# rayanirban/DiffSplitting

Measured on AMD Instinct MI355X. Metric: sampled images/sec (2000-step 128x128 SR3), higher is better.
Workload: dtype bf16; 1 GPU; sr_sr3_16_128: GaussianDiffusion.p_sample_loop, 16->128 SR3 UNet (97.8M params), T=2000 linear schedule; one step = UNet forward + posterior update of the batch; batch_per_gpu=16, global_batch=16, image=128x128x3, sample_steps=2000, parallelism=1 independent replicas, final RCCL all-gather, hipgraph=True, streams=1, noise=device Philox4x32-10, weights=random-init, seed 0

## Files before the change

diffsplitting_amd/csrc/dsx_conv_variants.h:

```cpp
#pragma once
#include "dsx_conv_common.h"

#ifndef DSX_RING_DEPTH
#define DSX_RING_DEPTH 6
#endif
#ifndef DSX_WS_DEPTH_EXPR
#define DSX_WS_DEPTH_EXPR (bm == 64 ? 5 : (bm == 256 ? 2 : (ks == 1 ? 3 : 4)))
#endif
#ifndef DSX_WS_DEPTH_C2_64
#define DSX_WS_DEPTH_C2_64 3
#endif
#ifndef DSX_RING_1X1_NB1
#define DSX_RING_1X1_NB1 16
#endif
#ifndef DSX_RING_1X1_NB2
#define DSX_RING_1X1_NB2 4
#endif

namespace dsx {

template <typename DT, int MB, int WM, int WN, int KS, int S, int CPG, int D, int MAX_IT>
__global__ __launch_bounds__(256, ((KS == 3 && CPG == 2) ? 2
                                  : (MB == 1 ? (S == 2 ? 3 : 4) : (MB == 2 ? 3 : (MB == 4 ? 2 : 1))))) void k_conv_mfma(const ConvArgs a);
template <typename DT, int MB, int WM, int WN, int NB, int KS, int CPG, int D, int NIT, int P, int LW>
__global__ __launch_bounds__(256 + 64 * LW, 1) void k_conv_ws(const ConvArgs a);
template <typename DT, int KS, int NPH> __global__ __launch_bounds__(512, 1) void k_conv_img(const ConvArgs a);

enum ConvFamily { FAM_MFMA, FAM_WS, FAM_IMG };
struct ConvVariant {
  int family, dtype, tile, ks, stride, cpg;
  void (*kern)(const ConvArgs);
  int block, lds_cap;
  int MB, WM, WN, NB;
  int max_px;
  int nit;
  int depth, nbuf;
  bool fuses_stats;
};
static constexpr int kLdsDefault = 64 * 1024, kLdsMax = 160 * 1024;
static constexpr int conv_cpg(int ks) { return ks == 1 ? 2 : 1; }

static constexpr int mfma_max_px(int bm, int ks, int stride, int cpg) {
  if (ks == 1) return bm;
  if (stride == 2) return 400;
  if (cpg == 2) return bm == 256 ? 324 : 220;
  return bm == 256 ? 400 : (bm == 128 ? 220 : 144);
}
template <typename DT, int TILE, int MB, int WM, int WN, int KS, int S = 1, int CPG = conv_cpg(KS)>
constexpr ConvVariant mfma_row() {
  constexpr bool G2 = KS == 3 && CPG == 2;
  constexpr int D = KS == 1 ? 4 : (G2 ? 6 : DSX_RING_DEPTH);
  constexpr int PX = mfma_max_px(32 * MB * WM, KS, S, CPG);
  constexpr int MI = (PX * 4 * CPG + 255) / 256;
  return {FAM_MFMA, Kind<DT>::value, TILE, KS, S, CPG, k_conv_mfma<DT, MB, WM, WN, KS, S, CPG, D, MI>, 256,
          G2 ? kLdsMax : kLdsDefault, MB, WM, WN, 1, PX, MI, 0, 2, MB <= 2};
}

static constexpr int kWsLoaderWaves = 4;
static constexpr int ws_max_px(int bm, int ks) { return ks == 1 ? bm : (bm == 256 ? 324 : (bm == 128 ? 180 : 108)); }
static constexpr int ws_depth(int bm, int ks, int cpg) {
  if (ks == 3 && cpg == 2) return bm == 64 ? DSX_WS_DEPTH_C2_64 : 2;
  if (ks == 3 && cpg == 4) return 1;
  if (ks == 1 && cpg == 4) return bm == 64 ? 2 : 1;
  return DSX_WS_DEPTH_EXPR;
}

#ifndef DSX_WS_NBUF_EXPR
#define DSX_WS_NBUF_EXPR(bm, ks, nb, cpg) ((bm) == 256 && (ks) == 3 ? 3 : 2)
#endif
static constexpr int ws_nbuf(int bm, int ks, int nb, int cpg) { return DSX_WS_NBUF_EXPR(bm, ks, nb, cpg); }

template <typename DT, int TILE, int MB, int WM, int WN, int NB, int KS, int CPG = conv_cpg(KS)>
constexpr ConvVariant ws_row() {
  constexpr int BM = 32 * MB * WM;
  constexpr int D = KS == 1 ? ((NB == 2 || MB == 4) ? DSX_RING_1X1_NB2 : DSX_RING_1X1_NB1) : ((NB == 2 || MB == 4) ? 6 : 18);
  constexpr int PX = ws_max_px(BM, KS);
  constexpr int NIT = (PX * 4 * CPG + kWsLoaderWaves * 64 - 1) / (kWsLoaderWaves * 64);
  constexpr int P = ws_depth(BM, KS, CPG);
  return {FAM_WS, Kind<DT>::value, TILE, KS, 1, CPG, k_conv_ws<DT, MB, WM, WN, NB, KS, CPG, D, NIT, P, kWsLoaderWaves>,
          256 + 64 * kWsLoaderWaves, kLdsMax, MB, WM, WN, NB, PX, NIT, P, ws_nbuf(BM, KS, NB, CPG), true};
}

template <typename DT, int KS, int NPH> constexpr ConvVariant img_row() {
  return {FAM_IMG, Kind<DT>::value, -1, KS, 1, NPH, k_conv_img<DT, KS, NPH>, 512, kLdsMax, 0, 0, 0, 0, 0, 0, 0, 0, true};
}

template <int N> struct ConvVariants {
  ConvVariant row[N];
  constexpr const ConvVariant* begin() const { return row; }
  constexpr const ConvVariant* end() const { return row + N; }
};
template <int... N> constexpr ConvVariants<(N + ...)> concat(const ConvVariants<N>&... parts) {
  ConvVariants<(N + ...)> out{};
  int n = 0;
  auto append = [&](const auto& p) { for (const ConvVariant& v : p) out.row[n++] = v; };
  (append(parts), ...);
  return out;
}

template <typename DT> constexpr ConvVariants<34> variants_of() {
  return {{
      mfma_row<DT, TILE_256x128, 8, 1, 4, 1>(), mfma_row<DT, TILE_256x128, 8, 1, 4, 3>(),
      mfma_row<DT, TILE_128x128, 4, 1, 4, 1>(), mfma_row<DT, TILE_128x128, 4, 1, 4, 3>(),
      mfma_row<DT, TILE_64x128, 2, 1, 4, 1>(), mfma_row<DT, TILE_64x128, 2, 1, 4, 3>(),
      mfma_row<DT, TILE_256x64, 4, 2, 2, 1>(), mfma_row<DT, TILE_256x64, 4, 2, 2, 3>(),
      mfma_row<DT, TILE_128x64, 2, 2, 2, 1>(), mfma_row<DT, TILE_128x64, 2, 2, 2, 3>(),
      mfma_row<DT, TILE_128x64, 2, 2, 2, 3, 1, 2>(),
      mfma_row<DT, TILE_64x64, 1, 2, 2, 1>(), mfma_row<DT, TILE_64x64, 1, 2, 2, 3>(),
      mfma_row<DT, TILE_64x64, 1, 2, 2, 3, 2>(),
      mfma_row<DT, TILE_128x32, 1, 4, 1, 1>(), mfma_row<DT, TILE_128x32, 1, 4, 1, 3>(),
      mfma_row<DT, TILE_128x32, 1, 4, 1, 3, 1, 2>(), mfma_row<DT, TILE_256x32, 2, 4, 1, 3, 1, 2>(),
      ws_row<DT, TILE_64x128, 2, 1, 4, 1, 1>(), ws_row<DT, TILE_64x128, 2, 1, 4, 1, 3>(),
      ws_row<DT, TILE_64x128, 2, 1, 4, 1, 1, 4>(),
      ws_row<DT, TILE_64x128, 2, 1, 4, 1, 3, 2>(),
      ws_row<DT, TILE_64x128, 2, 1, 4, 1, 3, 4>(),
      ws_row<DT, TILE_128x64, 2, 2, 2, 1, 1>(), ws_row<DT, TILE_128x64, 2, 2, 2, 1, 3>(),
      ws_row<DT, TILE_256x64, 4, 2, 2, 1, 3>(),
      ws_row<DT, TILE_64x64, 1, 2, 2, 1, 1>(), ws_row<DT, TILE_64x64, 1, 2, 2, 1, 3>(),
      img_row<DT, 1, 2>(), img_row<DT, 1, 4>(), img_row<DT, 1, 8>(),
      img_row<DT, 3, 2>(), img_row<DT, 3, 4>(), img_row<DT, 3, 8>(),
  }};
}
template <typename DT> constexpr ConvVariants<4> ws_nb2_variants() {
  return {{ws_row<DT, TILE_128x128, 2, 2, 2, 2, 1>(), ws_row<DT, TILE_128x128, 2, 2, 2, 2, 3>(),
           ws_row<DT, TILE_128x128, 2, 2, 2, 2, 1, 4>(), ws_row<DT, TILE_128x128, 2, 2, 2, 2, 3, 2>()}};
}
static constexpr auto kVariants = concat(variants_of<float>(), variants_of<__bf16>(), variants_of<_Float16>(),
                                         ws_nb2_variants<__bf16>(), ws_nb2_variants<_Float16>());

static constexpr int kKeySlots = 3 * 3 * (TILE_COUNT + 1) * 2 * 2 * 4;
static constexpr int key_slot(int family, int dtype, int tile, int ks, int stride, int cpg) {
  const int c = cpg == 1 ? 0 : (cpg == 2 ? 1 : (cpg == 4 ? 2 : (cpg == 8 ? 3 : -1)));
  if (family < 0 || family > FAM_IMG || dtype < 0 || dtype > 2 || tile < -1 || tile >= TILE_COUNT || (ks != 1 && ks != 3) ||
      (stride != 1 && stride != 2) || c < 0)
    return -1;
  return ((((family * 3 + dtype) * (TILE_COUNT + 1) + tile + 1) * 2 + ks / 2) * 2 + stride - 1) * 4 + c;
}
struct VariantIndex { short row[kKeySlots]; bool unique; };
static constexpr VariantIndex index_variants() {
  VariantIndex ix{};
  for (short& r : ix.row) r = -1;
  ix.unique = true;
  short n = 0;
  for (const ConvVariant& v : kVariants) {
    const int s = key_slot(v.family, v.dtype, v.tile, v.ks, v.stride, v.cpg);
    if (s < 0 || ix.row[s] >= 0) ix.unique = false;
    else ix.row[s] = n;
    ++n;
  }
  return ix;
}
static constexpr VariantIndex kIndex = index_variants();
static const ConvVariant* find_variant(int family, int dtype, int tile, int ks, int stride, int cpg) {
  const int s = key_slot(family, dtype, tile, ks, stride, cpg);
  return s >= 0 && kIndex.row[s] >= 0 ? &kVariants.row[kIndex.row[s]] : nullptr;
}

static int patch_pixels(int ks, int stride, const ConvArgs& a) {
  const int TW = 1 << a.tw_log2, TH = 1 << a.th_log2;
  return (((TH - 1) * stride + ks) * ((TW - 1) * stride + ks)) << a.tb_log2;
}
static hipError_t launch_variant(const ConvVariant& v, unsigned grid, size_t lds, const ConvArgs& a, hipStream_t st) {
  void* args[] = {(void*)&a};
  (void)hipLaunchKernel((const void*)v.kern, dim3(grid), dim3((unsigned)v.block), args, lds, st);
  return hipGetLastError();
}

}
```

diffsplitting_amd/csrc/dsx_conv_ws.hip:

```cpp
#include "dsx_conv_variants.h"
#include <algorithm>

#ifndef DSX_PRE_RESID_EXPR
#define DSX_PRE_RESID_EXPR (NB == 1 && MB <= 2)
#endif
#ifndef DSX_PFF_EXPR
#define DSX_PFF_EXPR (NB == 2 ? 3 : 6)
#endif
#ifndef DSX_WS_K0_EXPR
#define DSX_WS_K0_EXPR 64
#endif
#ifndef DSX_EPI_PRIO_COND
#define DSX_EPI_PRIO_COND false
#endif
#ifndef DSX_STAMP_CVT_COND
#define DSX_STAMP_CVT_COND (tiC == 2 && gC == 0)
#endif
#ifndef DSX_LOADER_PRIO
#define DSX_LOADER_PRIO 3
#endif
#ifndef DSX_LOADER_PRIO_EXPR
#define DSX_LOADER_PRIO_EXPR DSX_LOADER_PRIO
#endif

// ... 3 lines not shown
  for (int spin = 0; spin < (1 << 18); ++spin) {
    f32x4_t v;
    asm volatile("ds_read_b128 %0, %1\n\ts_waitcnt lgkmcnt(0)" : "=v"(v) : "v"(addr) : "memory");
    const int4 c = __builtin_bit_cast(int4, v);
    const int m = min(min(c.x, c.y), min(c.z, c.w));
    if (__builtin_amdgcn_readfirstlane(m) >= target) return;
    __builtin_amdgcn_s_sleep(1);
  }
  if (timeouts != nullptr && (threadIdx.x & 63) == 0) atomicAdd(timeouts, 1u);
}
static __device__ __forceinline__ void lds_signal(unsigned addr, int wave, int count) {
  asm volatile("s_waitcnt lgkmcnt(0)" ::: "memory");
  if ((threadIdx.x & 63) == 0) asm volatile("ds_write_b32 %0, %1" ::"v"(addr + 4u * (unsigned)wave), "v"(count) : "memory");
}

template <typename DT, int MB, int WM, int WN, int NB, int KS, int CPG, int D, int NIT, int P, int LW>
__global__ void k_conv_ws(const ConvArgs a) {
  constexpr int LT = 64 * LW;
  constexpr int S = 1;
  constexpr int KC = Chunk<DT>::KC;
  constexpr int CPU = Unit<DT>::N;
  constexpr int ES = (int)sizeof(DT);
  constexpr int UPP = KC / CPU;
  constexpr int UPG = UPP * CPG;
  constexpr int UPG_LOG2 = UPG == 16 ? 4 : (UPG == 8 ? 3 : 2);
  constexpr int UB = 16;
  constexpr int PIXB = 64 * CPG + 16;
  constexpr int TAPS = KS * KS;
  constexpr int PAD = KS / 2;
  constexpr int NSTEP = CPG * TAPS * 2;
  [[maybe_unused]] constexpr bool IS_BF16 = sizeof(DT) == 2;
  constexpr int RAWB = NIT * LT * 16;
  constexpr int NSLOT = P + 1;
  static_assert(D <= NSTEP ? NSTEP % D == 0 : (D % NSTEP == 0 && D / NSTEP <= 8), "ring depth divides the steps per group, or is a multiple of them");
  static_assert(WM * WN == 4 && P * NIT < 64, "4 compute waves; vmcnt is 6 bits");

  extern __shared__ __attribute__((aligned(16))) unsigned char lds[];

  const int tid = threadIdx.x;
  DSX_STAMP_T(63, tid == 0);
  const int lane = tid & 63;
  const int wave8 = __builtin_amdgcn_readfirstlane(tid >> 6);
  const bool loader = wave8 >= 4;
  const int wave = loader ? wave8 - 4 : wave8;
  const int ltid = loader ? tid - 256 : tid;
  const int c16 = lane & 15, kq = lane >> 4;

  const int TW = 1 << a.tw_log2, TH = 1 << a.th_log2;
  const int PW = (TW - 1) * S + KS;
  const int PH = (TH - 1) * S + KS;
  const int PPI = PH * PW;
  const int PP = PPI << a.tb_log2;
  const int RB = a.lds_row;
  const int BUFB = (PH << a.tb_log2) * RB;
  constexpr int NBUF = ws_nbuf(32 * MB * WM, KS, NB, CPG);
  static_assert(NBUF >= 2 && NBUF <= 4, "two images and a barrier, or three / four and counters");
  const int C = a.C0 + a.C1;
  const int AFFB = a.has_gn ? ((2 * C * 4 + 15) & ~15) : 0;
  float* const aff_base = (float*)(lds + NBUF * BUFB);
  unsigned char* const raw_base = lds + NBUF * BUFB + 3 * AFFB;
  const unsigned lds0 = (unsigned)(uintptr_t)(__attribute__((address_space(3))) unsigned char*)lds;
  const unsigned full_addr = lds0 + NBUF * BUFB + 3 * AFFB + NSLOT * RAWB;
  const int G = a.kchunks / CPG;

  const int wpn = a.ws_wg_per_n;
  int nt, p0;
  {
    const int bid = blockIdx.x, xcd = bid & 7, k = bid >> 3;
    if (a.ws_map == 0) {
      const int lg = a.ws_nt_log2, band = xcd >> lg;
      nt = xcd & ((1 << lg) - 1);
// ... 7 lines not shown
      const int j = (int)fastdiv((unsigned)k, a.mg_per);
      nt = k - j * a.ws_per;
      p0 = (j << 3) + xcd;
    } else {
      nt = (int)fastdiv((unsigned)bid, a.mg_wpn);
      p0 = bid - nt * wpn;
    }
  }
  const int ntile = wpn >= a.m_tiles ? (p0 < a.m_tiles ? 1 : 0)
                                     : (a.ws_bigdiv ? (a.m_tiles - p0 + wpn - 1) / wpn
                                                                : (int)fastdiv((unsigned)(a.m_tiles - p0 + wpn - 1), a.mg_wpn));
  const int total = ntile * G;

  if (loader) {
    __builtin_amdgcn_s_setprio(DSX_LOADER_PRIO_EXPR);
    struct TilePos { int tx, ty, b; };
    const int adv_x = a.ws_adv_x, adv_y = a.ws_adv_y, adv_b = a.ws_adv_b;
    auto tile_advance = [&](TilePos& t) __attribute__((always_inline)) {
      t.tx += adv_x;
      if (t.tx >= a.tiles_x) { t.tx -= a.tiles_x; t.ty += 1; }
      t.ty += adv_y;
      if (t.ty >= a.tiles_y) { t.ty -= a.tiles_y; t.b += 1; }
      t.b += adv_b;
    };
    auto tile_flags = [&](const TilePos& t) __attribute__((always_inline)) -> int {
      return (PAD == 0) ? 0
                        : ((t.ty == 0 ? 1 : 0) | (t.ty == a.tiles_y - 1 ? 2 : 0) | (t.tx == 0 ? 4 : 0) |
                           (t.tx == a.tiles_x - 1 ? 8 : 0));
    };
    auto tile_base = [&](const TilePos& t) __attribute__((always_inline)) -> int {
// ... 196 lines not shown
      if (++bufL == NBUF) bufL = 0;
      DSX_STAMP_T(66 + 4 * v, tid == 256 && v < 9);
      if (v + 2 < total) {
        wait_young(issued - (v + 3));
        fetch_next();
      }
      DSX_STAMP_T(67 + 4 * v, tid == 256 && v < 9);
      if constexpr (NBUF == 2) ws_barrier();
      DSX_STAMP_T(68 + 4 * v, tid == 256 && v < 9);
    }
    return;
  }

  const int wm = wave / WN, wn = wave % WN;
  const int pq = ws16_pixel(c16);
  int abase[MB][KS];
#pragma unroll
  for (int mb = 0; mb < MB; ++mb) {
    const int m = (wm * MB + mb) * 32 + pq;
    const int tx = m & (TW - 1);
    const int ty = (m >> a.tw_log2) & (TH - 1);
    const int tb = m >> (a.tw_log2 + a.th_log2);
#pragma unroll
    for (int dy = 0; dy < KS; ++dy)
      abase[mb][dy] = (tb * PH + ty * S + dy) * RB + tx * S * PIXB + ws16_slice(kq) * 16;
  }
  const int a16 = TW >= 32 ? 16 * S * PIXB : (16 >> a.tw_log2) * S * RB;
  const int blk0 = (nt * WN + wn) * NB;
  const int wblock = G * (NSTEP * 1024);
  const __amdgpu_buffer_rsrc_t rsw = __builtin_amdgcn_make_buffer_rsrc(
      (void*)((const unsigned char*)a.wpack + (size_t)blk0 * wblock), 0, NB * wblock, 0x00020000);
  const int wlane[2] = {ws16_woff(lane, 0), ws16_woff(lane, 1)};
  static_assert(D % 2 == 0 && NSTEP % 2 == 0, "ring slots alternate between the two fragments of a pair");
  const int qtot = G * NSTEP;
  int qn = 0;
  struct WFrag { uint4 v[NB]; };
  auto load_b = [&](auto chc) __attribute__((always_inline)) -> WFrag {
    constexpr int ch = decltype(chc)::value;
    WFrag f;
#pragma unroll
    for (int nb = 0; nb < NB; ++nb)
      f.v[nb] = __builtin_bit_cast(uint4, __builtin_amdgcn_raw_buffer_load_b128(rsw, wlane[ch], nb * wblock + (qn >> 1) * 2048, 0));
// ... 40 lines not shown
    return (t.b * a.Ho + (t.ty << a.th_log2)) * a.Wo + (t.tx << a.tw_log2);
  };
  TilePos cur;
  {
    const int q1 = (int)fastdiv((unsigned)p0, a.mg_tiles_x);
    cur.b = (int)fastdiv((unsigned)p0, a.mg_per_img);
    cur.tx = p0 - q1 * a.tiles_x;
    cur.ty = q1 - cur.b * a.tiles_y;
  }
  TilePos nxt = cur;
  tile_advance(nxt);
  TilePos nn = nxt;
  tile_advance(nn);

  auto load_aff = [&](int b, int slot) __attribute__((always_inline)) {
    if (a.gn_scale == nullptr || tid * 4 >= C) return;
    float* dst = aff_base + (size_t)slot * (AFFB / 4);
    *(float4*)(dst + tid * 4) = *(const float4*)(a.gn_scale + (size_t)b * C + tid * 4);
    *(float4*)(dst + C + tid * 4) = *(const float4*)(a.gn_shift + (size_t)b * C + tid * 4);
  };
  TilePos n3 = nn;
  tile_advance(n3);
  load_aff(cur.b, 0);
  if (ntile > 1) load_aff(nxt.b, 1);
  if (ntile > 2) load_aff(nn.b, 2);

  constexpr int NR = 8 / CPU;
  const float4 zero4 = make_float4(0.f, 0.f, 0.f, 0.f);
  float4 addv[NB][2], affv[2];
  constexpr bool PRE_RESID = DSX_PRE_RESID_EXPR;
  uint4 residv[PRE_RESID ? MB : 1][NB][2][NR];
// ... 25 lines not shown
          addv[nb][j] = *(const float4*)(a.film + (size_t)t.b * a.film_bs + nbase + 32 * nb + 4 * j);
    }
    if (PRE_RESID && a.resid) {
      const int r0 = tile_pixel0(t) * a.resid_ld;
#pragma unroll
      for (int mb = 0; mb < (PRE_RESID ? MB : 1); ++mb)
#pragma unroll
        for (int ph = 0; ph < 2; ++ph) {
          const DT* rp = (const DT*)a.resid + (r0 + rrow[mb] + ph * r16);
#pragma unroll
          for (int nb = 0; nb < NB; ++nb)
#pragma unroll
            for (int q = 0; q < NR; ++q) residv[mb][nb][ph][q] = *(const uint4*)(rp + 32 * nb + CPU * q);
        }
    }
    if (want_aff && a.gn_scale != nullptr && tid * 4 < C) {
      affv[0] = *(const float4*)(a.gn_scale + (size_t)b_aff * C + tid * 4);
      affv[1] = *(const float4*)(a.gn_shift + (size_t)b_aff * C + tid * 4);
    }
  };
  prefetch_epilogue(cur, ntile > 3, n3.b);

  constexpr bool PF_OK = !(NB == 2 && KS == 3);
  unsigned fin_pf_acc = 0u;
  if constexpr (PF_OK) fin_pf_acc = l2_prefetch_fold(l2_prefetch(a.pf, blockIdx.x, gridDim.x, tid, 256));
  if constexpr (KS == 1) {
    if (a.fin_on) {
      fin_pf_acc |= l2_prefetch_fold(l2_prefetch(a.fin.pf, blockIdx.x, gridDim.x, tid, 256));
      const int nitems = a.fin.B * a.fin.groups;
      for (int item = (int)blockIdx.x * 4 + wave; item < nitems; item += (int)gridDim.x * 4)
        gn_finalize_item<1>(a.fin, item % a.fin.B, item / a.fin.B, lane, nullptr);
// ... 25 lines not shown
    for (int v0 = 0; v0 < total; v0 += RP)
      static_for<RP>([&](auto rc_) __attribute__((always_inline)) {
        constexpr int R0 = decltype(rc_)::value * NSTEP;
        const int v = v0 + decltype(rc_)::value;
        if (v >= total) return;
#define DSX_WS_ITEM_NEXT return
#include "dsx_conv_ws_item.inc"
#undef DSX_WS_ITEM_NEXT
      });
  }
  if constexpr (PF_OK) l2_prefetch_retire(a.pf, fin_pf_acc);
}

static const ConvVariant* ws_variant(int dtype, int tile, int ks, const ConvArgs& a) {
  const int cpg = (ks == 3 && (a.ws_cpg == 2 || a.ws_cpg == 4)) ? a.ws_cpg : ((ks == 1 && a.ws_cpg == 4) ? 4 : conv_cpg(ks));
  return find_variant(FAM_WS, dtype, tile, ks, 1, cpg);
}
size_t conv_ws_lds_bytes(int dtype, int tile, int ks, const ConvArgs& a) {
  const ConvVariant* v = ws_variant(dtype, tile, ks, a);
  if (!v) return 0;
  const int cpg = v->cpg;
  if (cpg != conv_cpg(ks)) {
    const int gw = cpg * (dtype != 0 ? 32 : 16);
    if ((ks == 3 && a.cpg == 2) || a.kchunks % cpg || a.C0 % gw || a.C1 % gw) return 0;
    if ((1 << (a.tw_log2 + a.th_log2 + a.tb_log2)) != 32 * v->MB * v->WM) return 0;
    if (a.lds_row != conv_lds_row(ks, 1, a.tw_log2, cpg)) return 0;
  } else if (conv_lds_bytes(dtype, tile, ks, 1, a) == 0) return 0;
  if (patch_pixels(ks, 1, a) > v->max_px) return 0;
  if (a.up && (a.tw_log2 == 0 || a.th_log2 == 0)) return 0;
  const int ph = ((1 << a.th_log2) - 1) + ks;
  const size_t bufb = (size_t)(ph << a.tb_log2) * a.lds_row;
  const size_t rawb = (size_t)v->nit * (kWsLoaderWaves * 64 * 16);
  const size_t affb = a.has_gn ? (((size_t)2 * (a.C0 + a.C1) * 4 + 15) & ~(size_t)15) : 0;
  const size_t total = v->nbuf * bufb + 3 * affb + (size_t)(v->depth + 1) * rawb + (v->nbuf >= 3 ? 32 : 0);
  if (a.tb_log2 != 0 || a.kchunks / cpg < 2) return 0;
  if ((long long)a.B * a.Ho * a.Wo * std::max(a.out_ld, a.resid_ld) >= (1LL << 31)) return 0;
  const int al = dtype != 0 ? 7 : 3;
  if (a.Cout % (32 * v->WN * v->NB) != 0 || (a.out_ld & al) != 0 || (a.resid_ld & al) != 0 || a.C0 + a.C1 > 1024)
    return 0;
  if (dtype != 0 && !(a.act_bf16 && a.out_bf16)) return 0;
  return total <= (size_t)v->lds_cap ? total : 0;
}
hipError_t launch_conv_ws(int dtype, int tile, int ks, const ConvArgs& a, hipStream_t st) {
  const size_t lds = conv_ws_lds_bytes(dtype, tile, ks, a);
  if (lds == 0 || a.ksplit != 1 || a.ws_wg_per_n < 1 || a.stage_mode != 0) return hipErrorInvalidValue;
  if (a.bias && a.film) return hipErrorInvalidValue;
  return launch_variant(*ws_variant(dtype, tile, ks, a), (unsigned)(a.n_tiles * a.ws_wg_per_n), lds, a, st);
}

// ... 2 lines not shown
```

diffsplitting_amd/csrc/dsx_conv_ws_item.inc:

```
    unsigned aaddr[MB][KS];
#pragma unroll
    for (int mb = 0; mb < MB; ++mb)
#pragma unroll
      for (int dy = 0; dy < KS; ++dy) aaddr[mb][dy] = lds0 + ibuf * BUFB + abase[mb][dy];
    if constexpr (NBUF >= 3) lds_wait_all_ge(full_addr, v + 1, a.handoff_timeouts);
    f32x4_t fb[PFF + 1];
    auto read_frag = [&](auto kc_) __attribute__((always_inline)) {
      constexpr int k = decltype(kc_)::value;
      constexpr int t = k / NF, mb = (k % NF) >> 1, ph = k & 1;
      constexpr int cg = t / TAPS, tap = t % TAPS, dy = tap / KS, dx = tap % KS;
      constexpr int imm = dx * PIXB + cg * 64;
      static_assert(imm < 65536, "ds offset field");
#ifndef DSX_ABL_L
      lds_read_frag<imm>(fb[k % (PFF + 1)], ph ? aaddr[mb][dy] + (unsigned)a16 : aaddr[mb][dy]);
#else
      touch_frag(fb[k % (PFF + 1)], aaddr[mb][dy]);
#endif
    };
    static_for<PFF>(read_frag);
    static_for<NPAIR>([&](auto tc_) {
      constexpr int t = decltype(tc_)::value;
      constexpr int s0 = (R0 + 2 * t) % D, s1 = (R0 + 2 * t + 1) % D;
      const WFrag w0 = bq[s0], w1 = bq[s1];
#ifndef DSX_ABL_W
      bq[s0] = load_b(std::integral_constant<int, 0>{});
      bq[s1] = load_b(std::integral_constant<int, 1>{});
#endif
      static_for<NF>([&](auto fc_) __attribute__((always_inline)) {
        constexpr int f = decltype(fc_)::value, k = t * NF + f;
        constexpr int mb = f >> 1, ph = f & 1;
        if constexpr (k + PFF < FT) read_frag(std::integral_constant<int, k + PFF>{});
// ... 2 lines not shown
        const f32x4_t px = fb[k % (PFF + 1)];
#pragma unroll
        for (int nb = 0; nb < NB; ++nb) {
          f32x4_t q0 = {acc[mb][nb][8 * ph], acc[mb][nb][8 * ph + 1], acc[mb][nb][8 * ph + 2], acc[mb][nb][8 * ph + 3]};
          f32x4_t q1 = {acc[mb][nb][8 * ph + 4], acc[mb][nb][8 * ph + 5], acc[mb][nb][8 * ph + 6], acc[mb][nb][8 * ph + 7]};
          q0 = mfma16_step<DT>(w0.v[nb], px, q0);
          q1 = mfma16_step<DT>(w1.v[nb], px, q1);
#pragma unroll
          for (int j = 0; j < 4; ++j) { acc[mb][nb][8 * ph + j] = q0[j]; acc[mb][nb][8 * ph + 4 + j] = q1[j]; }
        }
      });
    });
    DSX_STAMP_T(1 + 3 * v, tid == 0 && v < 20);
    if constexpr (NBUF == 2) ws_barrier();
    else lds_signal(full_addr + 16, wave, v + 1);
    if (++ibuf == NBUF) ibuf = 0;
    DSX_STAMP_T(2 + 3 * v, tid == 0 && v < 20);
    if (++g < G) DSX_WS_ITEM_NEXT;
    g = 0;

    if (DSX_EPI_PRIO_COND) __builtin_amdgcn_s_setprio(2);
    if (a.gn_scale != nullptr && ti + 3 < ntile && tid * 4 < C) {
      float* dst = aff_base + (size_t)aslot * (AFFB / 4);
      *(float4*)(dst + tid * 4) = affv[0];
      *(float4*)(dst + C + tid * 4) = affv[1];
    }
    const int rcur = PRE_RESID ? 0 : tile_pixel0(cur) * a.resid_ld;
#pragma unroll
    for (int mb = 0; mb < MB; ++mb)
#pragma unroll
      for (int nb = 0; nb < NB; ++nb)
#pragma unroll
        for (int ph = 0; ph < 2; ++ph) {
          float rs[8];
#pragma unroll
          for (int q = 0; q < NR; ++q) {
            float t[CPU];
// ... 73 lines not shown
```

diffsplitting_amd/csrc/dsx_kernels.h:

```cpp
#pragma once
#include <hip/hip_runtime.h>
#include <stdint.h>

namespace dsx {

struct PrefetchArgs {
  const void* base;
  unsigned slice_bytes;
  int nslices;
  unsigned* sink;
};
inline unsigned fastdiv_magic(unsigned d) { return d <= 1 ? 0u : (unsigned)((1ull << 32) / d) + 1u; }
#if defined(__HIPCC__)
__device__ __forceinline__ unsigned fastdiv(unsigned n, unsigned magic) { return magic ? __umulhi(n, magic) : n; }
struct PfAcc { unsigned v[4]; };
__device__ __forceinline__ PfAcc l2_prefetch(const PrefetchArgs& pf, unsigned lin_block, unsigned nblocks_total, int tid, int nthreads) {
  PfAcc acc = {{0u, 0u, 0u, 0u}};
  if (pf.base == nullptr || pf.nslices <= 0) return acc;
  const unsigned label = lin_block & 7u, j = lin_block >> 3, n8 = (nblocks_total + 7u) >> 3;
  const unsigned lines = pf.slice_bytes >> 7;
  const unsigned per = (lines + n8 - 1u) / n8, l0 = j * per;
  const unsigned l1 = l0 + per < lines ? l0 + per : lines;
  const int s0 = pf.nslices < 8 ? (int)(label % (unsigned)pf.nslices) : (int)label;
  const int sstep = pf.nslices < 8 ? pf.nslices : 8;
// ... 148 lines not shown
  int tiles_x, tiles_y, m_tiles, n_tiles;
  int lds_row;
  int cpg;
  int ws_wg_per_n;
  int ws_cpg;
  int xcd_bands;
  int ws_map;
  int ws_nt_log2;
  int ws_per;
  int ws_adv_x, ws_adv_y, ws_adv_b;
  int ws_dpy, ws_dpx;
  unsigned mg_tiles_x, mg_per_img, mg_pw, mg_wpn, mg_per;
  int ws_bigdiv;
  float* stat_part;
  unsigned* handoff_timeouts;
  unsigned long long* stamp;
  int stamp_block;
  int ablate;
  const void* gn_part0; int gn_nchunk0, gn_pf32_0;
  const void* gn_part1; int gn_nchunk1, gn_pf32_1;
  StatPivot gn_piv0, gn_piv1;
  const float* gn_gamma; const float* gn_beta;
  int gn_groups; float gn_eps;
  PrefetchArgs pf;
  int fin_on;
  GnFinArgs fin;
  int ksplit;
  int groups_per_split;
  long long slab_stride;
};
// ... 395 lines not shown
```

diffsplitting_amd/csrc/dsx_plan.cpp:

```cpp
#include "dsx_rt.h"

static std::vector<int> tile_order(const char* e, const std::vector<int>& dflt) {
  if (!*e) return dflt;
  std::vector<int> v;
  for (const char* p = e; *p;) {
    v.push_back(atoi(p));
    while (*p && *p != ',') ++p;
    if (*p == ',') ++p;
  }
  return v;
}

PlanKnobs dsx::read_plan_knobs() {
  PlanKnobs k;
  static const struct { const char* name; int PlanKnobs::*field; } ints[] = {
      {"DSX_FIRST", &PlanKnobs::first}, {"DSX_IMG", &PlanKnobs::img}, {"DSX_WS", &PlanKnobs::ws},
      {"DSX_WS_1X1", &PlanKnobs::ws_1x1}, {"DSX_WS_MIN_GRID", &PlanKnobs::ws_min_grid}, {"DSX_WS_G2", &PlanKnobs::ws_g2},
      {"DSX_WS_G2_MIN64", &PlanKnobs::ws_g2_min64}, {"DSX_WS_G2_MIN128", &PlanKnobs::ws_g2_min128},
      {"DSX_WS_G4_MIN64", &PlanKnobs::ws_g4_min64}, {"DSX_WS_C4", &PlanKnobs::ws_c4},
      {"DSX_WS_C4_MIN", &PlanKnobs::ws_c4_min}, {"DSX_WS_MAP3", &PlanKnobs::ws_map3},
      {"DSX_XCD_BANDS", &PlanKnobs::xcd_bands}, {"DSX_HOST_FIN", &PlanKnobs::host_fin},
      {"DSX_PREFETCH", &PlanKnobs::prefetch}, {"DSX_PREFETCH_WS", &PlanKnobs::prefetch_ws},
      {"DSX_FUSE_STATS", &PlanKnobs::fuse_stats}, {"DSX_NARROW_G2", &PlanKnobs::narrow_g2},
      {"DSX_MIN_GRID", &PlanKnobs::min_grid}, {"DSX_SPLITK", &PlanKnobs::splitk}, {"DSX_ATTN_CS", &PlanKnobs::attn_cs},
#ifdef DSX_DIAG
      {"DSX_ABLATE", &PlanKnobs::ablate},
#endif
  };
  static const struct { const char* name; std::vector<int> PlanKnobs::*field; } lists[] = {
      {"DSX_TILES_WIDE", &PlanKnobs::tiles_wide}, {"DSX_TILES_NARROW", &PlanKnobs::tiles_narrow},
      {"DSX_TILES_SLIM", &PlanKnobs::tiles_slim}, {"DSX_TILES_WIDE_SPLIT", &PlanKnobs::tiles_wide_split},
      {"DSX_TILES_NARROW_SPLIT", &PlanKnobs::tiles_narrow_split}, {"DSX_TILES_NARROW_G2", &PlanKnobs::tiles_narrow_g2},
      {"DSX_TILES_WS_WIDE", &PlanKnobs::tiles_ws_wide}, {"DSX_TILES_WS_WIDE_1X1", &PlanKnobs::tiles_ws_wide_1x1},
      {"DSX_TILES_WS_WIDE_1X1_RAW", &PlanKnobs::tiles_ws_wide_1x1_raw}, {"DSX_TILES_WS_NARROW", &PlanKnobs::tiles_ws_narrow},
  };
// ... 208 lines not shown
  return wpn;
}

static void decide_ws_chunks(const PlanKnobs& k, int dtype, int ks, int tile, ConvArgs& a) {
  auto take = [&](bool wanted, int cpg) {
    ConvArgs t = a;
    t.ws_cpg = cpg; t.lds_row = conv_lds_row(ks, 1, a.tw_log2, cpg);
    if (wanted && conv_ws_lds_bytes(dtype, tile, ks, t) != 0) { a.ws_cpg = cpg; a.lds_row = t.lds_row; }
  };
  if (ks == 3) {
    const int min_chunks = conv_tile_info(tile).BM == 64 ? k.ws_g2_min64 : k.ws_g2_min128;
    take(k.ws_g2 && a.kchunks >= min_chunks, 2);
    take(k.ws_g2 && a.kchunks >= k.ws_g4_min64, 4);
  }
  if (ks == 1) take(k.ws_c4 && a.kchunks >= k.ws_c4_min, 4);
}

static int decide_ws_startup(const PlanKnobs& k, int ks, ConvArgs& w) {
  w.xcd_bands = k.xcd_bands;
  w.ws_wg_per_n = ws_wg_per_n(w);
  const bool map3 = k.ws_map3 && ks == 1 && w.n_tiles >= 2 && w.n_tiles <= 32;
  if (map3) {
    int wpn3 = std::max(8, (256 / w.n_tiles) / 8 * 8);
    if (wpn3 > w.m_tiles) wpn3 = (w.m_tiles + 7) / 8 * 8;
    w.ws_wg_per_n = wpn3;
  }
  const int NT = w.n_tiles, wpn = w.ws_wg_per_n, per_img = w.tiles_x * w.tiles_y;
  w.ws_map = map3 ? 3 : ((NT <= 8 && 8 % NT == 0 && wpn % (8 / NT) == 0) ? 0 : ((NT % 8) == 0 ? 1 : 2));
  w.ws_nt_log2 = NT <= 8 ? ilog2(NT) : 0;
  w.ws_per = map3 ? NT : (NT >> 3);
// ... 514 lines not shown
```

diffsplitting_amd/csrc/dsx_rt.h:

```cpp
#pragma once
#include <hip/hip_runtime.h>

#include <algorithm>
#include <cmath>
#include <cstdarg>
#include <cstdio>
#include <cstdlib>
#include <cstring>
#include <memory>
#include <string>
#include <utility>
#include <vector>

#include "../../include/dsx.h"
#include "dsx_kernels.h"

using namespace dsx;

namespace dsx {

int fail(int code, const char* fmt, ...);
#define HIP_TRY(expr)                                                                     \
  do {                                                                                    \
    hipError_t e__ = (expr);                                                              \
// ... 69 lines not shown
};

struct PlanKnobs {
  bool conv_naive = false;
  int first = 1;
  int img = 1;
  int ws = 1;
  int ws_1x1 = 1;
  int ws_min_grid = 224;
  int ws_g2 = 1;
  int ws_g2_min64 = 12;
  int ws_g2_min128 = 4;
  int ws_g4_min64 = 16;
  int ws_c4 = 1;
  int ws_c4_min = 8;
  int ws_map3 = 1;
  int xcd_bands = 1;
  int host_fin = 1;
  int prefetch = 1;
  int prefetch_ws = 1;
  int fuse_stats = 1;
  int narrow_g2 = 1;
  int min_grid = 512;
  int splitk = 1;
  int attn_cs = 2;
  int stamp_op = -1;
  int stamp_block = 0;
  std::string plan_dump;
  int ablate = 0;
  std::vector<int> tiles_wide{TILE_128x128, TILE_64x128, TILE_64x64};
// ... 158 lines not shown
```

Before: 2.927 images/s.

## Add direct buffer-to-LDS loading path for 1x1 warp-specialized convs

Adds a DIRECT variant of the warp-specialized conv kernel for 1x1 convolutions without group-norm or swish. Loader waves issue buffer_load_lds straight into swizzled per-image LDS slots, with a deeper image ring instead of a raw staging area plus repack. Consumers read A fragments with XOR-swizzled addresses and skip the padded row layout. The planner enables it by default when the LDS size check passes. This adds template variants and complexity, and the deeper ring with vmcnt-based waiting may shift LDS use and occupancy.

```diff
diff --git a/diffsplitting_amd/csrc/dsx_conv_variants.h b/diffsplitting_amd/csrc/dsx_conv_variants.h
--- a/diffsplitting_amd/csrc/dsx_conv_variants.h
+++ b/diffsplitting_amd/csrc/dsx_conv_variants.h
@@ -22,7 +22,7 @@
 template <typename DT, int MB, int WM, int WN, int KS, int S, int CPG, int D, int MAX_IT>
 __global__ __launch_bounds__(256, ((KS == 3 && CPG == 2) ? 2
                                   : (MB == 1 ? (S == 2 ? 3 : 4) : (MB == 2 ? 3 : (MB == 4 ? 2 : 1))))) void k_conv_mfma(const ConvArgs a);
-template <typename DT, int MB, int WM, int WN, int NB, int KS, int CPG, int D, int NIT, int P, int LW>
+template <typename DT, int MB, int WM, int WN, int NB, int KS, int CPG, int D, int NIT, int P, int LW, bool DIRECT>
 __global__ __launch_bounds__(256 + 64 * LW, 1) void k_conv_ws(const ConvArgs a);
 template <typename DT, int KS, int NPH> __global__ __launch_bounds__(512, 1) void k_conv_img(const ConvArgs a);
 
@@ -36,6 +36,7 @@
   int nit;
   int depth, nbuf;
   bool fuses_stats;
+  bool direct;
 };
 static constexpr int kLdsDefault = 64 * 1024, kLdsMax = 160 * 1024;
 static constexpr int conv_cpg(int ks) { return ks == 1 ? 2 : 1; }
@@ -53,7 +54,7 @@
   constexpr int PX = mfma_max_px(32 * MB * WM, KS, S, CPG);
   constexpr int MI = (PX * 4 * CPG + 255) / 256;
   return {FAM_MFMA, Kind<DT>::value, TILE, KS, S, CPG, k_conv_mfma<DT, MB, WM, WN, KS, S, CPG, D, MI>, 256,
-          G2 ? kLdsMax : kLdsDefault, MB, WM, WN, 1, PX, MI, 0, 2, MB <= 2};
+          G2 ? kLdsMax : kLdsDefault, MB, WM, WN, 1, PX, MI, 0, 2, MB <= 2, false};
 }
 
 static constexpr int kWsLoaderWaves = 4;
@@ -70,19 +71,23 @@
 #endif
 static constexpr int ws_nbuf(int bm, int ks, int nb, int cpg) { return DSX_WS_NBUF_EXPR(bm, ks, nb, cpg); }
 
-template <typename DT, int TILE, int MB, int WM, int WN, int NB, int KS, int CPG = conv_cpg(KS)>
+static constexpr int ws_direct_images(int bm, int cpg) { return ws_depth(bm, 1, cpg) + 3; }
+
+template <typename DT, int TILE, int MB, int WM, int WN, int NB, int KS, int CPG = conv_cpg(KS), bool DIRECT = false>
 constexpr ConvVariant ws_row() {
   constexpr int BM = 32 * MB * WM;
   constexpr int D = KS == 1 ? ((NB == 2 || MB == 4) ? DSX_RING_1X1_NB2 : DSX_RING_1X1_NB1) : ((NB == 2 || MB == 4) ? 6 : 18);
   constexpr int PX = ws_max_px(BM, KS);
   constexpr int NIT = (PX * 4 * CPG + kWsLoaderWaves * 64 - 1) / (kWsLoaderWaves * 64);
-  constexpr int P = ws_depth(BM, KS, CPG);
-  return {FAM_WS, Kind<DT>::value, TILE, KS, 1, CPG, k_conv_ws<DT, MB, WM, WN, NB, KS, CPG, D, NIT, P, kWsLoaderWaves>,
-          256 + 64 * kWsLoaderWaves, kLdsMax, MB, WM, WN, NB, PX, NIT, P, ws_nbuf(BM, KS, NB, CPG), true};
+  static_assert(!DIRECT || (KS == 1 && NB == 1), "direct rows: 1 x 1 convs, one N block per wave");
+  constexpr int NIMG = DIRECT ? ws_direct_images(BM, CPG) : ws_nbuf(BM, KS, NB, CPG);
+  constexpr int P = DIRECT ? NIMG - 1 : ws_depth(BM, KS, CPG);
+  return {FAM_WS, Kind<DT>::value, TILE, KS, 1, CPG, k_conv_ws<DT, MB, WM, WN, NB, KS, CPG, D, NIT, P, kWsLoaderWaves, DIRECT>,
+          256 + 64 * kWsLoaderWaves, kLdsMax, MB, WM, WN, NB, PX, NIT, P, NIMG, true, DIRECT};
 }
 
 template <typename DT, int KS, int NPH> constexpr ConvVariant img_row() {
-  return {FAM_IMG, Kind<DT>::value, -1, KS, 1, NPH, k_conv_img<DT, KS, NPH>, 512, kLdsMax, 0, 0, 0, 0, 0, 0, 0, 0, true};
+  return {FAM_IMG, Kind<DT>::value, -1, KS, 1, NPH, k_conv_img<DT, KS, NPH>, 512, kLdsMax, 0, 0, 0, 0, 0, 0, 0, 0, true, false};
 }
 
 template <int N> struct ConvVariants {
@@ -98,7 +103,7 @@
   return out;
 }
 
-template <typename DT> constexpr ConvVariants<34> variants_of() {
+template <typename DT> constexpr ConvVariants<37> variants_of() {
   return {{
       mfma_row<DT, TILE_256x128, 8, 1, 4, 1>(), mfma_row<DT, TILE_256x128, 8, 1, 4, 3>(),
       mfma_row<DT, TILE_128x128, 4, 1, 4, 1>(), mfma_row<DT, TILE_128x128, 4, 1, 4, 3>(),
@@ -117,6 +122,8 @@
       ws_row<DT, TILE_128x64, 2, 2, 2, 1, 1>(), ws_row<DT, TILE_128x64, 2, 2, 2, 1, 3>(),
       ws_row<DT, TILE_256x64, 4, 2, 2, 1, 3>(),
       ws_row<DT, TILE_64x64, 1, 2, 2, 1, 1>(), ws_row<DT, TILE_64x64, 1, 2, 2, 1, 3>(),
+      ws_row<DT, TILE_64x128, 2, 1, 4, 1, 1, 2, true>(), ws_row<DT, TILE_64x128, 2, 1, 4, 1, 1, 4, true>(),
+      ws_row<DT, TILE_128x64, 2, 2, 2, 1, 1, 2, true>(),
       img_row<DT, 1, 2>(), img_row<DT, 1, 4>(), img_row<DT, 1, 8>(),
       img_row<DT, 3, 2>(), img_row<DT, 3, 4>(), img_row<DT, 3, 8>(),
   }};
@@ -128,13 +135,13 @@
 static constexpr auto kVariants = concat(variants_of<float>(), variants_of<__bf16>(), variants_of<_Float16>(),
                                          ws_nb2_variants<__bf16>(), ws_nb2_variants<_Float16>());
 
-static constexpr int kKeySlots = 3 * 3 * (TILE_COUNT + 1) * 2 * 2 * 4;
-static constexpr int key_slot(int family, int dtype, int tile, int ks, int stride, int cpg) {
+static constexpr int kKeySlots = 3 * 3 * (TILE_COUNT + 1) * 2 * 2 * 4 * 2;
+static constexpr int key_slot(int family, int dtype, int tile, int ks, int stride, int cpg, bool direct) {
   const int c = cpg == 1 ? 0 : (cpg == 2 ? 1 : (cpg == 4 ? 2 : (cpg == 8 ? 3 : -1)));
   if (family < 0 || family > FAM_IMG || dtype < 0 || dtype > 2 || tile < -1 || tile >= TILE_COUNT || (ks != 1 && ks != 3) ||
       (stride != 1 && stride != 2) || c < 0)
     return -1;
-  return ((((family * 3 + dtype) * (TILE_COUNT + 1) + tile + 1) * 2 + ks / 2) * 2 + stride - 1) * 4 + c;
+  return (((((family * 3 + dtype) * (TILE_COUNT + 1) + tile + 1) * 2 + ks / 2) * 2 + stride - 1) * 4 + c) * 2 + (direct ? 1 : 0);
 }
 struct VariantIndex { short row[kKeySlots]; bool unique; };
 static constexpr VariantIndex index_variants() {
@@ -143,7 +150,7 @@
   ix.unique = true;
   short n = 0;
   for (const ConvVariant& v : kVariants) {
-    const int s = key_slot(v.family, v.dtype, v.tile, v.ks, v.stride, v.cpg);
+    const int s = key_slot(v.family, v.dtype, v.tile, v.ks, v.stride, v.cpg, v.direct);
     if (s < 0 || ix.row[s] >= 0) ix.unique = false;
     else ix.row[s] = n;
     ++n;
@@ -151,8 +158,8 @@
   return ix;
 }
 static constexpr VariantIndex kIndex = index_variants();
-static const ConvVariant* find_variant(int family, int dtype, int tile, int ks, int stride, int cpg) {
-  const int s = key_slot(family, dtype, tile, ks, stride, cpg);
+static const ConvVariant* find_variant(int family, int dtype, int tile, int ks, int stride, int cpg, bool direct = false) {
+  const int s = key_slot(family, dtype, tile, ks, stride, cpg, direct);
   return s >= 0 && kIndex.row[s] >= 0 ? &kVariants.row[kIndex.row[s]] : nullptr;
 }
 
diff --git a/diffsplitting_amd/csrc/dsx_conv_ws.hip b/diffsplitting_amd/csrc/dsx_conv_ws.hip
--- a/diffsplitting_amd/csrc/dsx_conv_ws.hip
+++ b/diffsplitting_amd/csrc/dsx_conv_ws.hip
@@ -41,7 +41,7 @@
   if ((threadIdx.x & 63) == 0) asm volatile("ds_write_b32 %0, %1" ::"v"(addr + 4u * (unsigned)wave), "v"(count) : "memory");
 }
 
-template <typename DT, int MB, int WM, int WN, int NB, int KS, int CPG, int D, int NIT, int P, int LW>
+template <typename DT, int MB, int WM, int WN, int NB, int KS, int CPG, int D, int NIT, int P, int LW, bool DIRECT>
 __global__ void k_conv_ws(const ConvArgs a) {
   constexpr int LT = 64 * LW;
   constexpr int S = 1;
@@ -52,7 +52,7 @@
   constexpr int UPG = UPP * CPG;
   constexpr int UPG_LOG2 = UPG == 16 ? 4 : (UPG == 8 ? 3 : 2);
   constexpr int UB = 16;
-  constexpr int PIXB = 64 * CPG + 16;
+  constexpr int PIXB = DIRECT ? 64 * CPG : 64 * CPG + 16;
   constexpr int TAPS = KS * KS;
   constexpr int PAD = KS / 2;
   constexpr int NSTEP = CPG * TAPS * 2;
@@ -79,9 +79,11 @@
   const int PPI = PH * PW;
   const int PP = PPI << a.tb_log2;
   const int RB = a.lds_row;
-  const int BUFB = (PH << a.tb_log2) * RB;
+  const int BUFB = DIRECT ? 32 * MB * WM * PIXB : (PH << a.tb_log2) * RB;
   constexpr int NBUF = ws_nbuf(32 * MB * WM, KS, NB, CPG);
   static_assert(NBUF >= 2 && NBUF <= 4, "two images and a barrier, or three / four and counters");
+  constexpr int NIMG = DIRECT ? P + 1 : NBUF;
+  static_assert(!DIRECT || (KS == 1 && NBUF == 2 && NIT * LT == 32 * MB * WM * UPG), "direct: 1 x 1, one barrier per item, whole DMA instructions");
   const int C = a.C0 + a.C1;
   const int AFFB = a.has_gn ? ((2 * C * 4 + 15) & ~15) : 0;
   float* const aff_base = (float*)(lds + NBUF * BUFB);
@@ -119,6 +121,83 @@
 
   if (loader) {
     __builtin_amdgcn_s_setprio(DSX_LOADER_PRIO_EXPR);
+    if constexpr (DIRECT) {
+      const int pix0 = ltid >> UPG_LOG2;
+      const int srcu = (ltid & (UPG - 1)) ^ (CPG == 4 ? (pix0 & 15) : ((pix0 >> 1) & 7));
+      int rel[NIT];
+#pragma unroll
+      for (int it = 0; it < NIT; ++it) {
+        const int m = pix0 + it * (LT >> UPG_LOG2);
+        rel[it] = (m >> a.tw_log2) * a.Ws + (m & (TW - 1));
+      }
+      const __amdgpu_buffer_rsrc_t rs0 = __builtin_amdgcn_make_buffer_rsrc(
+          (void*)a.src0, 0, (int)min((long long)a.B * a.Hs * a.Ws * a.C0 * ES, 0x7fffffffLL), 0x00020000);
+      const __amdgpu_buffer_rsrc_t rs1 = __builtin_amdgcn_make_buffer_rsrc(
+          (void*)(a.src1 ? a.src1 : a.src0), 0,
+          a.src1 ? (int)min((long long)a.B * a.Hs * a.Ws * a.C1 * ES, 0x7fffffffLL) : 0, 0x00020000);
+      const int adv_x = a.ws_adv_x, adv_y = a.ws_adv_y, adv_b = a.ws_adv_b;
+      int tx, ty, tb;
+      {
+        const int q1 = (int)fastdiv((unsigned)p0, a.mg_tiles_x);
+        tb = (int)fastdiv((unsigned)p0, a.mg_per_img);
+        tx = p0 - q1 * a.tiles_x;
+        ty = q1 - tb * a.tiles_y;
+      }
+      auto tile_base = [&]() __attribute__((always_inline)) -> int {
+        return (tb * a.Hs + (ty << a.th_log2)) * a.Ws + (tx << a.tw_log2);
+      };
+      int baseI = tile_base(), gI = 0, issued = 0, bufI = 0;
+      auto issue_next = [&]() __attribute__((always_inline)) {
+        const int c = gI * (CPG * KC) + srcu * CPU;
+        const bool first = gI * (CPG * KC) < a.C0;
+        const int cs = first ? a.C0 : a.C1;
+        const unsigned coff = c < C ? (unsigned)((first ? c : c - a.C0) * ES) : 0x80000000u;
+        unsigned char* dst = lds + bufI * BUFB + wave * 1024;
+#pragma unroll
+        for (int it = 0; it < NIT; ++it) {
+          const unsigned vo = c < C ? (unsigned)(baseI + rel[it]) * (unsigned)(cs * ES) + coff : 0x80000000u;
+          auto ldst = (__attribute__((address_space(3))) void*)(dst + it * (LT * 16));
+          if (first) __builtin_amdgcn_raw_ptr_buffer_load_lds(rs0, ldst, 16, vo, 0, 0, 0);
+          else __builtin_amdgcn_raw_ptr_buffer_load_lds(rs1, ldst, 16, vo, 0, 0, 0);
+        }
+        ++issued;
+        if (++bufI == NIMG) bufI = 0;
+        if (++gI == G) {
+          gI = 0;
+          tx += adv_x;
+          if (tx >= a.tiles_x) { tx -= a.tiles_x; ty += 1; }
+          ty += adv_y;
+          if (ty >= a.tiles_y) { ty -= a.tiles_y; tb += 1; }
+          tb += adv_b;
+          baseI = tile_base();
+        }
+      };
+      auto wait_young = [&](int young) __attribute__((always_inline)) {
+        if (young >= P) wait_vmcnt<P * NIT>();
+        else static_for<P>([&](auto jc) __attribute__((always_inline)) {
+          if (young == decltype(jc)::value) wait_vmcnt<decltype(jc)::value * NIT>();
+        });
+        __builtin_amdgcn_sched_barrier(0);
+      };
+      DSX_STAMP_T(110, tid == 256);
+      while (issued < NIMG && issued < total) issue_next();
+      DSX_STAMP_T(111, tid == 256);
+      ws_barrier();
+      if (total > 0) wait_young(issued - 1);
+      DSX_STAMP_T(112, tid == 256);
+      ws_barrier();
+      DSX_STAMP_T(64, tid == 256);
+      for (int v = 0; v < total; ++v) {
+        DSX_STAMP_T(65 + 4 * v, tid == 256 && v < 9);
+        DSX_STAMP_T(66 + 4 * v, tid == 256 && v < 9);
+        if (v + 1 < total) wait_young(issued - (v + 2));
+        DSX_STAMP_T(67 + 4 * v, tid == 256 && v < 9);
+        ws_barrier();
+        DSX_STAMP_T(68 + 4 * v, tid == 256 && v < 9);
+        if (issued < total) issue_next();
+      }
+      return;
+    }
     struct TilePos { int tx, ty, b; };
     const int adv_x = a.ws_adv_x, adv_y = a.ws_adv_y, adv_b = a.ws_adv_b;
     auto tile_advance = [&](TilePos& t) __attribute__((always_inline)) {
@@ -345,18 +424,25 @@
 
   const int wm = wave / WN, wn = wave % WN;
   const int pq = ws16_pixel(c16);
-  int abase[MB][KS];
+  constexpr int AD = DIRECT ? CPG : KS;
+  int abase[MB][AD];
 #pragma unroll
   for (int mb = 0; mb < MB; ++mb) {
     const int m = (wm * MB + mb) * 32 + pq;
+    if constexpr (DIRECT) {
+      const int sg = CPG == 4 ? (m & 15) : ((m >> 1) & 7);
+#pragma unroll
+      for (int cg = 0; cg < AD; ++cg) abase[mb][cg] = m * PIXB + (((cg * 4 + ws16_slice(kq)) ^ sg) << 4);
+      continue;
+    }
     const int tx = m & (TW - 1);
     const int ty = (m >> a.tw_log2) & (TH - 1);
     const int tb = m >> (a.tw_log2 + a.th_log2);
 #pragma unroll
     for (int dy = 0; dy < KS; ++dy)
-      abase[mb][dy] = (tb * PH + ty * S + dy) * RB + tx * S * PIXB + ws16_slice(kq) * 16;
-  }
-  const int a16 = TW >= 32 ? 16 * S * PIXB : (16 >> a.tw_log2) * S * RB;
+      abase[mb][DIRECT ? 0 : dy] = (tb * PH + ty * S + dy) * RB + tx * S * PIXB + ws16_slice(kq) * 16;
+  }
+  const int a16 = DIRECT ? 16 * PIXB : (TW >= 32 ? 16 * S * PIXB : (16 >> a.tw_log2) * S * RB);
   const int blk0 = (nt * WN + wn) * NB;
   const int wblock = G * (NSTEP * 1024);
   const __amdgpu_buffer_rsrc_t rsw = __builtin_amdgcn_make_buffer_rsrc(
@@ -427,7 +513,7 @@
   tile_advance(nn);
 
   auto load_aff = [&](int b, int slot) __attribute__((always_inline)) {
-    if (a.gn_scale == nullptr || tid * 4 >= C) return;
+    if (DIRECT || a.gn_scale == nullptr || tid * 4 >= C) return;
     float* dst = aff_base + (size_t)slot * (AFFB / 4);
     *(float4*)(dst + tid * 4) = *(const float4*)(a.gn_scale + (size_t)b * C + tid * 4);
     *(float4*)(dst + C + tid * 4) = *(const float4*)(a.gn_shift + (size_t)b * C + tid * 4);
@@ -483,7 +569,7 @@
             for (int q = 0; q < NR; ++q) residv[mb][nb][ph][q] = *(const uint4*)(rp + 32 * nb + CPU * q);
         }
     }
-    if (want_aff && a.gn_scale != nullptr && tid * 4 < C) {
+    if (!DIRECT && want_aff && a.gn_scale != nullptr && tid * 4 < C) {
       affv[0] = *(const float4*)(a.gn_scale + (size_t)b_aff * C + tid * 4);
       affv[1] = *(const float4*)(a.gn_shift + (size_t)b_aff * C + tid * 4);
     }
@@ -539,7 +625,7 @@
 
 static const ConvVariant* ws_variant(int dtype, int tile, int ks, const ConvArgs& a) {
   const int cpg = (ks == 3 && (a.ws_cpg == 2 || a.ws_cpg == 4)) ? a.ws_cpg : ((ks == 1 && a.ws_cpg == 4) ? 4 : conv_cpg(ks));
-  return find_variant(FAM_WS, dtype, tile, ks, 1, cpg);
+  return find_variant(FAM_WS, dtype, tile, ks, 1, cpg, a.ws_direct != 0);
 }
 size_t conv_ws_lds_bytes(int dtype, int tile, int ks, const ConvArgs& a) {
   const ConvVariant* v = ws_variant(dtype, tile, ks, a);
@@ -557,7 +643,9 @@
   const size_t bufb = (size_t)(ph << a.tb_log2) * a.lds_row;
   const size_t rawb = (size_t)v->nit * (kWsLoaderWaves * 64 * 16);
   const size_t affb = a.has_gn ? (((size_t)2 * (a.C0 + a.C1) * 4 + 15) & ~(size_t)15) : 0;
-  const size_t total = v->nbuf * bufb + 3 * affb + (size_t)(v->depth + 1) * rawb + (v->nbuf >= 3 ? 32 : 0);
+  if (v->direct && (ks != 1 || a.has_gn || a.swish || a.up)) return 0;
+  const size_t total = v->direct ? (size_t)v->nbuf * (32 * v->MB * v->WM) * (64 * cpg)
+                                 : v->nbuf * bufb + 3 * affb + (size_t)(v->depth + 1) * rawb + (v->nbuf >= 3 ? 32 : 0);
   if (a.tb_log2 != 0 || a.kchunks / cpg < 2) return 0;
   if ((long long)a.B * a.Ho * a.Wo * std::max(a.out_ld, a.resid_ld) >= (1LL << 31)) return 0;
   const int al = dtype != 0 ? 7 : 3;
diff --git a/diffsplitting_amd/csrc/dsx_conv_ws_item.inc b/diffsplitting_amd/csrc/dsx_conv_ws_item.inc
--- a/diffsplitting_amd/csrc/dsx_conv_ws_item.inc
+++ b/diffsplitting_amd/csrc/dsx_conv_ws_item.inc
@@ -1,20 +1,21 @@
-    unsigned aaddr[MB][KS];
+    unsigned aaddr[MB][AD];
 #pragma unroll
     for (int mb = 0; mb < MB; ++mb)
 #pragma unroll
-      for (int dy = 0; dy < KS; ++dy) aaddr[mb][dy] = lds0 + ibuf * BUFB + abase[mb][dy];
+      for (int dy = 0; dy < AD; ++dy) aaddr[mb][dy] = lds0 + ibuf * BUFB + abase[mb][dy];
     if constexpr (NBUF >= 3) lds_wait_all_ge(full_addr, v + 1, a.handoff_timeouts);
     f32x4_t fb[PFF + 1];
     auto read_frag = [&](auto kc_) __attribute__((always_inline)) {
       constexpr int k = decltype(kc_)::value;
       constexpr int t = k / NF, mb = (k % NF) >> 1, ph = k & 1;
       constexpr int cg = t / TAPS, tap = t % TAPS, dy = tap / KS, dx = tap % KS;
-      constexpr int imm = dx * PIXB + cg * 64;
+      constexpr int imm = DIRECT ? 0 : dx * PIXB + cg * 64;
+      constexpr int ai = DIRECT ? cg : dy;
       static_assert(imm < 65536, "ds offset field");
 #ifndef DSX_ABL_L
-      lds_read_frag<imm>(fb[k % (PFF + 1)], ph ? aaddr[mb][dy] + (unsigned)a16 : aaddr[mb][dy]);
+      lds_read_frag<imm>(fb[k % (PFF + 1)], ph ? aaddr[mb][ai] + (unsigned)a16 : aaddr[mb][ai]);
 #else
-      touch_frag(fb[k % (PFF + 1)], aaddr[mb][dy]);
+      touch_frag(fb[k % (PFF + 1)], aaddr[mb][ai]);
 #endif
     };
     static_for<PFF>(read_frag);
@@ -47,13 +48,13 @@
     DSX_STAMP_T(1 + 3 * v, tid == 0 && v < 20);
     if constexpr (NBUF == 2) ws_barrier();
     else lds_signal(full_addr + 16, wave, v + 1);
-    if (++ibuf == NBUF) ibuf = 0;
+    if (++ibuf == NIMG) ibuf = 0;
     DSX_STAMP_T(2 + 3 * v, tid == 0 && v < 20);
     if (++g < G) DSX_WS_ITEM_NEXT;
     g = 0;
 
     if (DSX_EPI_PRIO_COND) __builtin_amdgcn_s_setprio(2);
-    if (a.gn_scale != nullptr && ti + 3 < ntile && tid * 4 < C) {
+    if (!DIRECT && a.gn_scale != nullptr && ti + 3 < ntile && tid * 4 < C) {
       float* dst = aff_base + (size_t)aslot * (AFFB / 4);
       *(float4*)(dst + tid * 4) = affv[0];
       *(float4*)(dst + C + tid * 4) = affv[1];
diff --git a/diffsplitting_amd/csrc/dsx_kernels.h b/diffsplitting_amd/csrc/dsx_kernels.h
--- a/diffsplitting_amd/csrc/dsx_kernels.h
+++ b/diffsplitting_amd/csrc/dsx_kernels.h
@@ -186,6 +186,7 @@
   int ws_bigdiv;
   float* stat_part;
   unsigned* handoff_timeouts;
+  int ws_direct;
   unsigned long long* stamp;
   int stamp_block;
   int ablate;
diff --git a/diffsplitting_amd/csrc/dsx_plan.cpp b/diffsplitting_amd/csrc/dsx_plan.cpp
--- a/diffsplitting_amd/csrc/dsx_plan.cpp
+++ b/diffsplitting_amd/csrc/dsx_plan.cpp
@@ -18,7 +18,7 @@
       {"DSX_WS_1X1", &PlanKnobs::ws_1x1}, {"DSX_WS_MIN_GRID", &PlanKnobs::ws_min_grid}, {"DSX_WS_G2", &PlanKnobs::ws_g2},
       {"DSX_WS_G2_MIN64", &PlanKnobs::ws_g2_min64}, {"DSX_WS_G2_MIN128", &PlanKnobs::ws_g2_min128},
       {"DSX_WS_G4_MIN64", &PlanKnobs::ws_g4_min64}, {"DSX_WS_C4", &PlanKnobs::ws_c4},
-      {"DSX_WS_C4_MIN", &PlanKnobs::ws_c4_min}, {"DSX_WS_MAP3", &PlanKnobs::ws_map3},
+      {"DSX_WS_C4_MIN", &PlanKnobs::ws_c4_min}, {"DSX_WS_DIRECT", &PlanKnobs::ws_direct}, {"DSX_WS_MAP3", &PlanKnobs::ws_map3},
       {"DSX_XCD_BANDS", &PlanKnobs::xcd_bands}, {"DSX_HOST_FIN", &PlanKnobs::host_fin},
       {"DSX_PREFETCH", &PlanKnobs::prefetch}, {"DSX_PREFETCH_WS", &PlanKnobs::prefetch_ws},
       {"DSX_FUSE_STATS", &PlanKnobs::fuse_stats}, {"DSX_NARROW_G2", &PlanKnobs::narrow_g2},
@@ -257,6 +257,11 @@
     take(k.ws_g2 && a.kchunks >= k.ws_g4_min64, 4);
   }
   if (ks == 1) take(k.ws_c4 && a.kchunks >= k.ws_c4_min, 4);
+  if (ks == 1 && k.ws_direct && !a.has_gn && !a.swish) {
+    ConvArgs t = a;
+    t.ws_direct = 1;
+    if (conv_ws_lds_bytes(dtype, tile, ks, t) != 0) a.ws_direct = 1;
+  }
 }
 
 static int decide_ws_startup(const PlanKnobs& k, int ks, ConvArgs& w) {
diff --git a/diffsplitting_amd/csrc/dsx_rt.h b/diffsplitting_amd/csrc/dsx_rt.h
--- a/diffsplitting_amd/csrc/dsx_rt.h
+++ b/diffsplitting_amd/csrc/dsx_rt.h
@@ -107,6 +107,7 @@
   int ws_g4_min64 = 16;
   int ws_c4 = 1;
   int ws_c4_min = 8;
+  int ws_direct = 1;
   int ws_map3 = 1;
   int xcd_bands = 1;
   int host_fin = 1;
```

Result: faster. 2.960 images/s (median of 6 runs) (+1.1%).
